# InteractiveComputerGraphics/stark

Measured on AMD Instinct MI355X. Metric: Newton-steps/s, higher is better.
Workload: dtype f64

## Files before the change

stark_amd/csrc/api.cpp:

```cpp
#include <algorithm>
#include <chrono>
#include <cstring>
#include <cstdio>
#include <cstdlib>
#include <string>

#include "dist.hpp"
#include "engine.hpp"
#include "forces.hpp"
#include "../../include/mistark_contact.h"

using namespace mistark;

#define API_BEGIN        \
    if (!ctx) return -1; \
    int _ret = 0;        \
    (void)_ret;          \
    ::mistark::DryScope _dry(ctx->c.dry); \
    try {                \
        if (!ctx->c.dry) (void)hipSetDevice(ctx->c.device);
#define API_END(ret)                   \
    }                                  \
    catch (const std::exception& e)    \
    {                                  \
// ... 445 lines not shown
    API_BEGIN
    ctx->c.touch();
    ctx->c.u_version++;
    Context& c = ctx->c;
    if (potential < 0 || potential >= (int)c.pots.size()) throw Error("bad potential id");
    const int part = dynamic ? 1 : 0;
    if (c.pots[potential].part != part) {
        c.pots[potential].part = part;
        c.layout_dirty = true;
        c.part[0].dirty = c.part[1].dirty = true;
    }
    API_END(0)
}
int mistark_potential_update_connectivity(mistark_ctx* ctx, int potential, const int32_t* conn, int32_t n_elem)
{
    API_BEGIN
    ctx->c.touch_potential(potential);
    Context& c = ctx->c;
    if (potential < 0 || potential >= (int)c.pots.size()) throw Error("bad potential id");
    if (n_elem < 0) throw Error("bad connectivity shape");
    Potential& P = c.pots[potential];
    P.n_elem = n_elem;
    P.conn_host.assign(conn, conn + (size_t)n_elem * P.conn_stride);
    P.conn_dirty = true;
    c.layout_dirty = true;
    API_END(0)
}

int64_t mistark_ndofs(mistark_ctx* ctx)
{
    if (!ctx) return -1;
    int64_t n = 0;
    for (auto& s : ctx->c.dof_sets) n += s.n;
    return n;
}
int mistark_get_dofs(mistark_ctx* ctx, double* u_host)
{
    API_BEGIN
    Context& c = ctx->c;
    prepare(c);
    MS_CHECK(hipMemcpyAsync(u_host, c.u.p, (size_t)c.ndofs * sizeof(double), hipMemcpyDeviceToHost, c.stream));
    MS_CHECK(hipStreamSynchronize(c.stream));
    API_END(0)
}
int mistark_set_dofs(mistark_ctx* ctx, const double* u_host)
{
    API_BEGIN
    ctx->c.touch();
    ctx->c.u_version++;
    Context& c = ctx->c;
    prepare(c);
    MS_CHECK(hipMemcpyAsync(c.u.p, u_host, (size_t)c.ndofs * sizeof(double), hipMemcpyHostToDevice, c.stream));
    MS_CHECK(hipStreamSynchronize(c.stream));
    API_END(0)
}
int64_t mistark_custom_emit(const char* name, const int32_t* strides, int32_t n_bindings, const int32_t* in_dof, const int32_t* ops, const double* constants, int32_t n_ops,
                            int32_t n_inputs, const int32_t* cond_ops, const double* cond_constants, int32_t n_cond_ops, int32_t n_blocks, int32_t compile, char* out, int64_t cap)
{
    try {
        if (!name || !strides || !in_dof || !ops || !constants) throw Error("mistark_custom_emit: null argument");
        size_t code = 0;
        const std::string src = custom_emit_source(name, strides, n_bindings, in_dof, ops, constants, n_ops, n_inputs, cond_ops, cond_constants, n_cond_ops, n_blocks, compile != 0, &code);
        if (out && cap > 0) std::snprintf(out, (size_t)cap, "%s", src.c_str());
        return compile ? (int64_t)code : (int64_t)src.size();
    } catch (const std::exception& e) {
        if (out && cap > 0) std::snprintf(out, (size_t)cap, "%s", e.what());
        return -1;
    }
}
int mistark_get_counter(mistark_ctx* ctx, const char* name, int64_t* out)
{
    API_BEGIN
    Context& c = ctx->c;
    if (!name || !out) throw Error("mistark_get_counter: null argument");
    const std::string n = name;
    if (n == "multi_pgh_launches") *out = c.n_multi_pgh;
    else if (n == "dof_skips_verified") *out = c.n_dof_skips_verified;
    else if (n == "rtc_builds") *out = c.n_rtc_builds;
    else if (n == "custom_kernel_us") *out = (int64_t)c.custom_kernel_us;
    else if (n == "rtc_launches") *out = c.n_rtc_launches;
    else if (n == "rtc_build_ms") *out = (int64_t)(1e3 * c.t_rtc_builds);
    else if (n == "fused_solves") *out = c.n_fused_solves;
    else if (n == "unfused_solves") *out = c.n_unfused_solves;
    else if (n == "evt_tet_us") *out = (int64_t)c.evt_sum[1];
    else if (n == "evt_small_us") *out = (int64_t)c.evt_sum[2];
    else if (n == "evt_gather_us") *out = (int64_t)c.evt_sum[3];
    else if (n == "evt_main_us") *out = (int64_t)c.evt_sum[4];
    else if (n == "evt_pattern_us") *out = (int64_t)c.evt_sum[5];
    else if (n == "evt_n") *out = c.evt_n;
    else if (n == "eval_pgh_issue_us") *out = (int64_t)(1e6 * c.t_eval_issue);
    else if (n == "eval_pgh_wait_us") *out = (int64_t)(1e6 * c.t_eval_wait);
    else if (n == "contact_searches") *out = contact_searches(c, false);
    else if (n == "contact_repeated_searches") *out = contact_searches(c, true);
    else if (n == "ccd_queries") *out = contact_ccd_counter(c, 0);
    else if (n == "ccd_skipped_pairs") *out = contact_ccd_counter(c, 1);
    else if (n == "ccd_capped_pairs") *out = contact_ccd_counter(c, 2);
    else if (n == "ccd_rounds") *out = contact_ccd_counter(c, 3);
    else if (n == "ccd_pad_bound_pairs") *out = contact_ccd_counter(c, 4);
    else if (n == "asm_short_slots_0" || n == "asm_short_slots_1") { ensure_pattern(c); const BsrPart& m = c.part[n.back() - '0']; *out = m.nnzb - m.n_long - m.n_vlong; }
    else if (n == "asm_long_slots_0" || n == "asm_long_slots_1") { ensure_pattern(c); *out = c.part[n.back() - '0'].n_long; }
    else if (n == "asm_vlong_slots_0" || n == "asm_vlong_slots_1") { ensure_pattern(c); *out = c.part[n.back() - '0'].n_vlong; }
    else if (n == "force_readouts") *out = c.n_force_readouts;
    else if (n == "force_long_rows") *out = force_long_rows(c);
    else if (n == "stress_readouts") *out = c.n_stress_readouts;
    else if (n == "stress_long_rows") *out = stress_long_rows(c);
    else if (n == "budget_readouts") *out = c.n_budget_readouts;
    else if (n == "budget_chunks") *out = c.n_budget_chunks;
    else if (n == "constraint_reports") *out = c.n_constraint_reports;
    else if (n == "constraint_report_chunks") *out = c.n_constraint_chunks;
    else if (n == "bending_reports") *out = c.n_bending_reports;
    else if (n == "bending_report_long_rows") *out = bending_long_rows(c);
    else if (n == "bending_report_chunks") *out = c.n_bending_chunks;
    else if (n == "spectrum_reports") *out = c.n_spectrum_reports;
    else if (n == "spectrum_report_long_rows") *out = spectrum_long_rows(c);
    else if (n == "spectrum_report_chunks") *out = c.n_spectrum_chunks;
    else if (n == "linsys_reports") *out = c.n_linsys_reports;
    else if (n == "wrench_reports") *out = c.n_wrench_reports;
    else if (n == "wrench_long_rows") *out = wrench_long_rows(c);
    else if (n == "contact_reports") *out = c.n_contact_reports;
    else if (n == "contact_report_long_rows") *out = contact_report_long_rows(c);
    else if (n == "friction_reports") *out = c.n_friction_reports;
    else if (n == "friction_report_long_rows") *out = friction_report_long_rows(c);
    else if (n == "llt_path") *out = c.llt_last_path;
    else if (n == "llt_panel_rows") *out = c.llt_last_panel_rows;
    else if (n == "llt_panels") *out = c.llt_last_panels;
    else if (n == "llt_fronts") *out = c.llt_last_fronts;
    else throw Error("mistark_get_counter: unknown counter '" + n + "'");
    API_END(0)
}
int mistark_dofs_to_host_arrays(mistark_ctx* ctx)
{
    API_BEGIN
    Context& c = ctx->c;
    prepare(c);
    for (auto& s : c.dof_sets)
        if (s.n > 0) MS_CHECK(hipMemcpyAsync(s.host, c.u.p + s.offset, s.n * sizeof(double), hipMemcpyDeviceToHost, c.stream));
    MS_CHECK(hipStreamSynchronize(c.stream));
    c.u_host_version = c.u_version;
    API_END(0)
}
int mistark_dofs_to_host_arrays_if_changed(mistark_ctx* ctx)
{
    API_BEGIN
    Context& c = ctx->c;
    prepare(c);
    if (c.u_host_version != c.u_version) {
        for (auto& s : c.dof_sets)
            if (s.n > 0) MS_CHECK(hipMemcpyAsync(s.host, c.u.p + s.offset, s.n * sizeof(double), hipMemcpyDeviceToHost, c.stream));
        MS_CHECK(hipStreamSynchronize(c.stream));
        c.u_host_version = c.u_version;
    } else {
        static const bool verify = [] { const char* e = std::getenv("MISTARK_VERIFY_DOF_SKIP"); return e && e[0] == '1'; }();
        if (verify) {
            std::vector<double> tmp;
            for (auto& s : c.dof_sets) {
                if (s.n <= 0) continue;
                tmp.resize((size_t)s.n);
                MS_CHECK(hipMemcpyAsync(tmp.data(), c.u.p + s.offset, s.n * sizeof(double), hipMemcpyDeviceToHost, c.stream));
                MS_CHECK(hipStreamSynchronize(c.stream));
                if (std::memcmp(tmp.data(), s.host, (size_t)s.n * sizeof(double)) != 0)
                    throw Error("mistark_dofs_to_host_arrays_if_changed: the transfer was skipped (version " + std::to_string(c.u_version) + ") but DoF set '" + s.label +
                                "' differs between the device and the caller's array: a writer of the DoF vector did not bump Context::u_version");
            }
            c.n_dof_skips_verified++;
        }
    }
// ... 769 lines not shown
    } catch (const std::exception& e) {
        comm->last_error = e.what();
        return -1;
    }
}
int mistark_rccl_allreduce_bench(int device, int rank, int world, const char unique_id[128], int64_t n_big, int reps, double* out, char* err, int err_len)
{
    if (!unique_id || !out) return -1;
    try {
        rccl_allreduce_bench(device, rank, world, unique_id, (size_t)std::max<int64_t>(n_big, 0), reps, out);
        return 0;
    } catch (const std::exception& e) {
        if (err && err_len > 0) std::snprintf(err, (size_t)err_len, "%s", e.what());
        return -1;
    }
}
int mistark_dist_fused_bench(mistark_ctx* ctx, int n_launches, double* out)
{
    API_BEGIN
    Context& c = ctx->c;
    if (c.world < 2 || !c.coll || !c.coll->ipc()) throw Error("mistark_dist_fused_bench: ranks that exchange through windows only");
    if (!out || n_launches <= 0) throw Error("mistark_dist_fused_bench: bad arguments");
    fused_pcg_replay(c, n_launches, &out[0], &out[1]);
    API_END(0)
}
mistark_local_group* mistark_local_group_create(int world)
{
    if (world < 1) return nullptr;
    auto* g = new mistark_local_group();
    g->g = std::make_shared<LocalGroup>(world);
    return g;
}
void mistark_local_group_destroy(mistark_local_group* g) { delete g; }
int mistark_dist_init_local(mistark_ctx* ctx, mistark_local_group* group, int rank)
{
    API_BEGIN
    if (!group) throw Error("null group");
    set_dist(ctx->c, rank, group->g->world, group->g->world > 1 ? make_local_collective(group->g, rank, ctx->c.device) : nullptr);
    API_END(0)
}

int mistark_set_option(mistark_ctx* ctx, const char* name, int value)
{
    API_BEGIN
    const std::string n = name ? name : "";
    if (n == "force_generic") {
        ctx->c.force_generic = value != 0;
        ctx->c.layout_dirty = true;
    }
    else if (n == "generic_contact") ctx->c.generic_contact = value != 0;
    else if (n == "no_eval_prelaunch") ctx->c.no_eval_prelaunch = value != 0;
    else if (n == "no_multi_eval_p") ctx->c.no_multi_eval_p = value != 0;
    else if (n == "no_multi_eval_pgh") ctx->c.no_multi_eval_pgh = value != 0;
    else if (n == "llt_multifrontal") ctx->c.llt_multifrontal = value;
    else if (n == "llt_no_coords") { ctx->c.llt_no_coords = value != 0; ctx->c.llt_mf_pattern_version = 0; }
    else if (n == "generic_inertia") ctx->c.generic_inertia = value != 0;
    else if (n == "contact_closed_min_lanes") ctx->c.contact_closed_min_lanes = value;
    else if (n == "atomic_assembly") ctx->c.atomic_assembly = value != 0;
    else if (n == "spmv_grid_cap") ctx->c.spmv_grid_cap = value;
    else if (n == "spmv_nt") ctx->c.spmv_nt = value;
    else if (n == "custom_rtc") ctx->c.custom_rtc = value;
    else if (n == "custom_timing") ctx->c.custom_timing = value;
    else if (n == "pcg_batch") ctx->c.pcg_batch = value;
    else if (n == "lazy_hessians") ctx->c.lazy_allowed = value != 0;
    else if (n == "lazy_eval") ctx->c.lazy_eval = value != 0;
    else if (n == "no_pattern_overlap") ctx->c.no_pattern_overlap = value != 0;
    else if (n == "no_eval_overlap") ctx->c.no_eval_overlap = value != 0;
    else if (n == "no_eager_assembly") ctx->c.no_eager_assembly = value != 0;
    else if (n == "no_sym_gather") ctx->c.no_sym_gather = value != 0;
    else if (n == "no_split_gather") ctx->c.no_split_gather = value != 0;
    else if (n == "no_bounded_pattern") { ctx->c.no_bounded_pattern = value != 0; ctx->c.part[1].dirty = true; }
    else if (n == "no_grad_gather") { ctx->c.no_grad_gather = value != 0; ctx->c.layout_dirty = true; }

    else if (n == "spmv_variant") ctx->c.spmv_variant = value;
    else if (n == "proj_variant") ctx->c.proj_variant = value;
    else if (n == "no_contact_cache") ctx->c.no_contact_cache = value != 0;
    else if (n == "no_sharded_search") ctx->c.no_sharded_search = value != 0;
    else if (n == "no_row_order") { ctx->c.no_row_order = value != 0; ctx->c.perm_sig.clear(); ctx->c.layout_dirty = true; }
    else if (n == "row_order") { ctx->c.row_order_mode = value; ctx->c.perm_sig.clear(); ctx->c.layout_dirty = true; }
    else if (n == "atomic_projection") ctx->c.atomic_projection = value != 0;
    else if (n == "no_dyn_pool") { ctx->c.no_dyn_pool = value != 0; ctx->c.layout_dirty = true; }
    else if (n == "no_halo_subset") { ctx->c.no_halo_subset = value != 0; ctx->c.cg_mask_pattern = 0; }
    else if (n == "cg_variant") ctx->c.cg_variant = value;
    else if (n == "no_fused_pcg") ctx->c.no_fused_pcg = value != 0;
    else if (n == "spmv_chunk_tiles") {
        if (value < 0 || value > 64) throw Error("spmv_chunk_tiles: 0 (automatic) .. 64");
        ctx->c.spmv_chunk_tiles = value;
        ctx->c.part[0].dirty = true;
    }
    else throw Error("unknown option '" + n + "'");
    API_END(0)
}

int mistark_sync(mistark_ctx* ctx)
{
    API_BEGIN
    MS_CHECK(hipStreamSynchronize(ctx->c.stream));
    API_END(0)
}
int mistark_spmv_bench(mistark_ctx* ctx, int n_launches, double* avg_us)
{
    API_BEGIN
    const double us = spmv_bench(ctx->c, n_launches);
    if (avg_us) *avg_us = us;
    API_END(0)
}

int mistark_spmv_event_overhead(mistark_ctx* ctx, double* avg_ms)
{
    API_BEGIN
    Context& c = ctx->c;
    if (avg_ms) *avg_ms = c.spmv_n > 0 ? c.spmv_empty_ms_sum / (double)c.spmv_n : 0.0;
    API_END(0)
}
int mistark_spmv_device_clock(mistark_ctx* ctx, double* avg_ms, int64_t* n)
{
    API_BEGIN
    Context& c = ctx->c;
    int khz = 0;
    MS_CHECK(hipDeviceGetAttribute(&khz, hipDeviceAttributeWallClockRate, c.device));
    if (khz <= 0) throw Error("spmv_device_clock: the device reports no wall clock rate");
    if (avg_ms) *avg_ms = c.spmv_clk_n > 0 ? c.spmv_clk_ticks / (double)c.spmv_clk_n / (double)khz : 0.0;
    if (n) *n = c.spmv_clk_n;
    API_END(0)
}
int mistark_spmv_timing(mistark_ctx* ctx, int reset, double* avg_ms, int64_t* n, double* bytes_per_launch)
{
    API_BEGIN
    Context& c = ctx->c;
    if (avg_ms) *avg_ms = c.spmv_n > 0 ? c.spmv_ms_sum / (double)c.spmv_n : 0.0;
    if (n) *n = c.spmv_n;
    if (bytes_per_launch)
        *bytes_per_launch = (double)(c.part[0].nnzb + c.part[1].nnzb) * 40.0 + ((double)c.nbr + 1.0) * 8.0 + 48.0 * (double)c.nbr + 56.0 * (double)c.part[1].n_rows;
    if (reset) {
        c.spmv_ms_sum = 0.0;
        c.spmv_empty_ms_sum = 0.0;
        c.spmv_n = 0;
        c.spmv_clk_ticks = 0.0;
        c.spmv_clk_n = 0;
        c.time_spmv = reset > 0;
    }
    API_END(0)
}

}

namespace mistark {
int force_potentials_by_prefix(mistark_ctx* ctx, const std::string& prefix, std::vector<int32_t>& out)
{
    API_BEGIN
    out.clear();
    for (size_t p = 0; p < ctx->c.pots.size(); p++)
        if (ctx->c.pots[p].name.compare(0, prefix.size(), prefix) == 0) out.push_back((int32_t)p);
    API_END(0)
}
int force_record(mistark_ctx* ctx, int slot, const std::vector<int32_t>& pots, double scale)
{
    API_BEGIN
    force_record_slot(ctx->c, slot, pots.data(), (int32_t)pots.size(), false, scale);
    API_END(0)
}
int force_fetch(mistark_ctx* ctx, int slot, double* f_host, int64_t ndofs)
{
    API_BEGIN
    force_fetch_slot(ctx->c, slot, f_host, ndofs);
    API_END(0)
// ... 160 lines not shown
```

stark_amd/csrc/engine.hpp:

```cpp
#pragma once
#include <algorithm>
#include <cstdlib>
#include <hip/hip_runtime.h>

#include <cstdint>
#include <cstdio>
#include <stdexcept>
#include <map>
#include <string>
#include <vector>

#include <memory>

#include "../../include/mistark.h"

#include "potargs.hpp"

namespace mistark {

struct Error : std::runtime_error
{
    using std::runtime_error::runtime_error;
};

// ... 535 lines not shown
    std::vector<ConstraintReportSet> cnr_slots;
    struct ConstraintPlan
    {
        DevBuf<uint32_t> items;
        DevBuf<int32_t> chunks;
        uint64_t conn_version = 0;
        int n_elem = -1, n_groups = -1;
        int64_t n_chunks = 0;
    };
    std::map<int, ConstraintPlan> cnr_plans;
    DevBuf<double> cnr_tol, cnr_partial;
    int64_t n_constraint_reports = 0;
    int64_t n_constraint_chunks = 0;

    DevBuf<double> bdr_rec, bdr_out, bdr_groups, bdr_thr, bdr_partial;
    DevBuf<uint32_t> bdr_key, bdr_key_alt, bdr_val, bdr_val_alt;
    DevBuf<uint32_t> bdr_stat;
    DevBuf<unsigned char> bdr_desc;
    DevBuf<uint8_t> bdr_cub_tmp;
    struct BendingPlan
    {
        DevBuf<uint32_t> items;
        DevBuf<int32_t> chunks;
        uint64_t conn_version = 0;
        int n_elem = -1, n_groups = -1;
        int64_t n_chunks = 0;
    };
    std::map<int, BendingPlan> bdr_plans;
    struct BendingSlot
    {
        DevBuf<double> rec, nodal, groups[2];
        int64_t N = -1;
        int64_t n_rows[2] = {0, 0}, col0[2] = {0, 0};
        int32_t n_groups = 0;
        int64_t nbr = 0;
    };
    BendingSlot bdr_slot;
    int64_t n_bending_reports = 0;
    int64_t n_bending_chunks = 0;
    bool bdr_stat_valid = false;

    DevBuf<double> wr_pool, wr_elemE, wr_f, wr_rec, wr_out;
    DevBuf<uint32_t> wr_key, wr_key_alt, wr_val, wr_val_alt;
    DevBuf<uint32_t> wr_stat;
    DevBuf<unsigned char> wr_desc;
    DevBuf<uint8_t> wr_cub_tmp, wr_active;
    DevBuf<int32_t> wr_ids, wr_count;
    int wr_stat_families = 0;
    int32_t wr_out_families = 0, wr_out_bodies = 0;
    int64_t n_wrench_reports = 0;

    DevBuf<double> spr_rec, spr_spec, spr_H, spr_gpool, spr_elemE, spr_nodal, spr_partial, spr_pot;
    DevBuf<uint32_t> spr_key, spr_key_alt, spr_val, spr_val_alt;
    DevBuf<uint32_t> spr_stat;
    DevBuf<unsigned char> spr_desc, spr_sdesc;
    DevBuf<uint8_t> spr_cub_tmp;
    DevBuf<int32_t> spr_chunks;
    struct SpectrumSlot
    {
        DevBuf<double> rec, nodal, pot;
        std::vector<int> slot_of;
        std::vector<int64_t> col0, n_elem;
        int64_t N = -1;
        int64_t nbr = 0;
    };
    SpectrumSlot spr_slot;
    int64_t n_spectrum_reports = 0;
    int64_t n_spectrum_chunks = 0;
    bool spr_stat_valid = false;

    DevBuf<double> lsr_V, lsr_w, lsr_t, lsr_y, lsr_part, lsr_c, lsr_ctrl, lsr_L, lsr_diag, lsr_nodal, lsr_q;
    DevBuf<uint8_t> lsr_nz;
    DevBuf<int32_t> lsr_cols;
    int64_t n_linsys_reports = 0;
    struct LinsysSlot
    {
        bool valid = false;
        double rec[16] = {0};
        double low_row = -1.0, low_share = 0.0, high_row = -1.0, high_share = 0.0;
    };
    LinsysSlot lsr_slot;

    int last_cg_iters = 0;
    int64_t n_projected_total = 0;

    ~Context();
};

void direct_mf_destroy(void* multifrontal);
void fetch(Context& c, void* dst_host, const void* src_dev, size_t bytes);
void h2d_staged(Context& c, void* dst_dev, const void* src_host, size_t bytes);
constexpr int FILL_BATCH_MAX = 8;
struct FillQueue
{
    hipStream_t stream;
    void* ptr[FILL_BATCH_MAX];
    size_t words[FILL_BATCH_MAX];
    uint32_t value[FILL_BATCH_MAX];
    int n = 0;
    explicit FillQueue(hipStream_t s) : stream(s) {}
    ~FillQueue() { flush(); }
    void add(void* p, int byte_value, size_t bytes);
    void flush();
};
void fill_async(hipStream_t stream, void* p, int byte_value, size_t bytes);
void copy_async(hipStream_t stream, void* dst, const void* src, size_t bytes);
void prepare(Context& c);
void eval_prelaunch(Context& c, int mode, bool lazy);
void shard_prepare(Context& c);
void shard_halo(Context& c, double* v_local);
void shard_halo_global(Context& c, double* v_global);
void shard_gather_global(Context& c, const double* v_local, double* v_global);
void shard_to_local(Context& c, const double* v_global, double* v_local, bool with_ghosts);
void shard_allgather_scalars(Context& c, const double* mine, int n, double* all_host);
double shard_sum(Context& c, double mine);
void shard_check(Context& c);
struct ElemTable
{
    const int32_t* rows;
    int64_t n_elem;
    int nb;
};
void rcb_partition_rows(int64_t n_block_rows, int world, const double* xyz, const std::vector<int64_t>& weight, std::vector<int32_t>& owner);
void graph_partition_rows(int64_t n_block_rows, int world, const std::vector<ElemTable>& tables, const uint8_t* hub, std::vector<int32_t>& owner);
void static_graph_order(Context& c, std::vector<int32_t>& rows_in_order);
void ensure_pattern(Context& c);
void contact_destroy(struct ContactSystem* cs);
int64_t contact_searches(const Context& c, bool repeated);
int64_t contact_ccd_counter(const Context& c, int which);
int64_t contact_sharded_searches(const Context& c);
void contact_shared_rows(Context& c, std::vector<int32_t>& rows);
struct ContactReportView
{
    const int32_t *cv_src, *cv_mesh, *tri, *tri_mesh, *edge, *edge_mesh, *mesh_kind;
    const double *thick, *k, *X_rest, *rb_xloc;
    const uint64_t* keys;
    int64_t n_keys;
    int bounds[22];
    int n_mesh, n_v, n_t, n_e;
    int prim_bits;
    const std::vector<int32_t>*h_tri, *h_cv_src, *h_cv_mesh;
};
void contact_report_view(Context& c, ContactReportView& v, bool sizes_only);
void contact_report_positions(Context& c, double* X_dev);
void contact_report_sizes(Context& c, int64_t* n_rows, int64_t* n_vertices, int32_t* n_groups);
void contact_report_run(Context& c, int set);
void contact_report_rows(Context& c, int set, int32_t* rows_i, double* rows_d, int64_t* n_rows);
void contact_report_vertices(Context& c, int set, double* out, int32_t* group, int32_t* source_index, int64_t* n_vertices);
void contact_report_pairs(Context& c, int set, double* out, int32_t* n_groups);
int64_t contact_report_long_rows(Context& c);
struct FrictionReportView
{
    struct Table
    {
        const int32_t* conn = nullptr;
        const double *T = nullptr, *mu = nullptr, *fn = nullptr, *bary = nullptr;
        int stride = 0, nbary = 0, start = 0, n = 0;
    };
    const int32_t *cv_src, *cv_mesh, *tri, *tri_mesh, *edge, *edge_mesh, *mesh_kind, *mesh_idx;
    const double *v1, *rb_v1, *rb_w1, *rb_q0, *rb_xloc;
    const uint64_t* keys;
    int64_t n_keys;
    Table tables[14];
    double dt, epsv;
    int n_mesh, n_v, n_t, n_e, prim_bits;
    const std::vector<int32_t>*h_tri, *h_cv_src, *h_cv_mesh;
};
void friction_report_view(Context& c, FrictionReportView& v, bool sizes_only);
void friction_report_sizes(Context& c, int64_t* n_rows, int64_t* n_vertices, int32_t* n_groups);
void friction_report_run(Context& c, int set);
void friction_report_rows(Context& c, int set, int32_t* rows_i, double* rows_d, int64_t* n_rows);
void friction_report_vertices(Context& c, int set, double* out, int32_t* group, int32_t* source_index, int64_t* n_vertices);
void friction_report_pairs(Context& c, int set, double* out, int32_t* n_groups);
int64_t friction_report_long_rows(Context& c);
int register_potential(Context& c, const char* name, const int32_t* conn, int32_t n_elem, int32_t conn_stride, const mistark_binding* bindings, int32_t n_bindings);
void eval(Context& c, int mode, double* E, double* grad_host, double* grad_max_abs = nullptr, bool lazy = false);
void reduce_dot_and_max_abs(Context& c, const double* a, const double* b, int64_t n, double* dot, double* max_abs_a);
void project(Context& c, double eps, int mirroring, const uint8_t* active_host, bool by_gradient, double threshold, int* all_active,
             int64_t* n_projected_now, int64_t* n_changed_now);
void assemble(Context& c);
void build_preconditioner(Context& c);
double spmv_bench(Context& c, int n);
void rows_from_solver(Context& c, const double* v_solver, double* v_caller);
void rows_to_solver(Context& c, const double* v_caller, double* v_solver);
void fused_pcg_replay(Context& c, int n_launches, double* s_us, double* v_us);
void spmv_device(Context& c, const double* x, double* y, const double* pdot, double* partials);
void pcg(Context& c, const double* rhs_dev, double abs_tol, double rel_tol, int max_iter, int stop_on_indef, mistark_pcg_info* info, double rhs_scale = 1.0);
bool direct_llt(Context& c, const double* rhs_dev, double* x_dev);
std::shared_ptr<CustomProgram> make_custom_program(const std::string& name, const int32_t* strides, int n_bindings, const int32_t* ops, const double* consts, int n_ops, int n_inputs,
                                                   const int32_t* cond_ops, const double* cond_consts, int n_cond_ops);
void custom_program_set_summation(CustomProgram& G, const std::string& name, int first_input, int stride, int n_iterations, const double* data);
void launch_eval_custom(Context& c, Potential& P, int mode);
void h2d_small(Context& c, void* dst_dev, const void* src_host, size_t bytes);
double reduce_max_abs(Context& c, const double* v, int64_t n);
double reduce_dot(Context& c, const double* a, const double* b, int64_t n);
void vec_axpby(Context& c, double* dst, double a, const double* x, double b, const double* y, int64_t n);
void vec_fill(Context& c, double* dst, double v, int64_t n);
void vec_neg(Context& c, double* dst, const double* x, int64_t n);
void launch_force_elements(Context& c, const Potential& P, double* pool, double* scratchE);
bool force_readout(Context& c, const int32_t* pots, int32_t n, bool all, double scale, double* f_dev);
void force_elements_host(Context& c, int pot, double scale, double* out, int32_t* block_rows, int64_t* n_elem, int32_t* nb);
void force_nodal_host(Context& c, const int32_t* pots, int32_t n, double scale, double* f_host);
void force_resultant_host(Context& c, const int32_t* pots, int32_t n, double scale, const int32_t* rows, int64_t n_rows, const double* pos_host, const double* about, double* out);
int64_t force_long_rows(Context& c);
void force_record_slot(Context& c, int slot, const int32_t* pots, int32_t n, bool all, double scale);
void force_fetch_slot(Context& c, int slot, double* f_host, int64_t n);
void stress_elements_host(Context& c, int pot, double* out, int64_t* n_elem, int32_t* kind);
void stress_nodal_host(Context& c, const int32_t* pots, int32_t n, double* out_host);
int64_t stress_long_rows(Context& c);
void stress_record_kind(Context& c, int kind);
void stress_fetch_elements(Context& c, int kind, double* out, int64_t* n_elem);
void stress_fetch_nodal(Context& c, int kind, double* out, int64_t n_rows);
std::vector<int> select_potentials(Context& c, const int32_t* pots, int32_t n, bool all, const char* who);
void launch_energy_elements(Context& c, const Potential& P, double* scratchE);
void budget_energies(Context& c, const int32_t* pots, int32_t n, double* out_host, int slot);
void budget_inertia(Context& c, int pot, const double* about, int32_t n_groups, double* out_host, int slot);
void budget_rigid(Context& c, int t0, int q0, int v1, int w1, int mass, int J_loc, int32_t n_bodies, const double* about, double* out_host, int slot);
void budget_fetch_slot(Context& c, int slot, double* out_host, int64_t n);
void constraint_rows_host(Context& c, int pot, const double* tolerance, int32_t n_groups, double* out, double* aux, int32_t* ids, int64_t* n_rows, int32_t* kind);
void constraint_groups_host(Context& c, int pot, const double* tolerance, int32_t n_groups, const double* about, double* out);
void constraint_record_kind(Context& c, int pot, const double* tolerance, int32_t n_groups, const double* about, int32_t* kind);
void constraint_fetch_kind(Context& c, int kind, double* out, double* aux, int32_t* ids, double* groups, int64_t* n_rows, int32_t* n_groups);
void bending_rows_host(Context& c, int pot, const double* threshold, int32_t n_groups, double* out, int64_t* n_rows, int32_t* kind);
void bending_nodal_host(Context& c, const int32_t* pots, int32_t n, double* out_host);
void bending_groups_host(Context& c, int pot, const double* threshold, int32_t n_groups, double* out);
int64_t bending_long_rows(Context& c);
void bending_record_step(Context& c, int pot_complete, int pot_flat, const double* threshold, int32_t n_groups);
void bending_fetch_kind(Context& c, int kind, double* rows, double* groups, int64_t* n_rows, int32_t* n_groups);
void bending_fetch_nodal(Context& c, double* out, int64_t n_rows);
void launch_hessian_elements(Context& c, const Potential& P, double* Hpool, double* scratchE, double* scratch_gpool);
void spectrum_rows_host(Context& c, int pot, int source, double eps, double* out, double* spectrum, int64_t* n_elem, int32_t* nb);
void spectrum_nodal_host(Context& c, const int32_t* pots, int32_t n, int source, double eps, double* out_host);
void spectrum_pots_host(Context& c, const int32_t* pots, int32_t n, int source, double eps, double* out);
int64_t spectrum_long_rows(Context& c);
void spectrum_record_step(Context& c, const int32_t* pots, int32_t n, double eps);
void spectrum_fetch_summary(Context& c, int32_t n, double* pots_out, double* nodal_out, int64_t n_rows);
void spectrum_fetch_rows(Context& c, int32_t index, double* rows, int64_t* n_rows);
void linsys_report_host(Context& c, int op, int m, const double* start_host, double* out, double* ritz, double* tri, int32_t* k_out);
void linsys_modes_host(Context& c, int op, int m, const double* start_host, const int32_t* which, int32_t n_which, double* x_host, double* nodal, double* mode);
void linsys_potential_shares_host(Context& c, int op, int m, const double* start_host, int32_t which, const int32_t* pots, int32_t n, double* out);
void linsys_record_step(Context& c, int op, int m);
void linsys_fetch(Context& c, double* rec16, double* rows4);
void wrench_rows_host(Context& c, int pot, int v1, int w1, int t0, int q0, int32_t n_bodies, double* out, int32_t* ids, int64_t* n_rows);
void wrench_bodies_host(Context& c, const int32_t* families, const int32_t* family_start, int32_t n_families, int v1, int w1, int t0, int q0, int32_t n_bodies, const double* about,
                        double* out, int32_t* count);
int64_t wrench_long_rows(Context& c);
void wrench_record_step(Context& c, const std::vector<std::vector<int32_t>>& families, const std::vector<char>& all, int v1, int w1, int t0, int q0, int32_t n_bodies,
                        const double* about);
void wrench_fetch_step(Context& c, int32_t n_families, int32_t n_bodies, double* out, int32_t* count);
struct InertiaBindings
{
    const double *dt = nullptr, *gravity = nullptr;
};
InertiaBindings inertia_bindings(const Context& c);
int find_kind(const char* name);
int kind_nb(int kind);
int kind_nbind(int kind);
void kind_strides(int kind, int* out);
const char* kind_name(int kind);
int n_kinds();

int newton_solve(Context& c, const mistark_newton_settings& s, const mistark_newton_callbacks* cb, mistark_newton_stats& st);
// ... 10 lines not shown
```

stark_amd/csrc/newton.cpp:

```cpp
#include <algorithm>
#include <chrono>
#include <cmath>
#include <cstdio>
#include <cstdlib>
#include <limits>

#include "engine.hpp"

namespace mistark {

namespace {
struct Timer
{
    double& acc;
    std::chrono::steady_clock::time_point t0;
    explicit Timer(double& a) : acc(a), t0(std::chrono::steady_clock::now()) {}
    ~Timer() { acc += std::chrono::duration<double>(std::chrono::steady_clock::now() - t0).count(); }
};
enum Stage { ST_EVAL_PGH, ST_EVAL_P, ST_ASSEMBLY, ST_PROJECT, ST_SOLVE, ST_OTHER, ST_COUNT };
struct GpuStages
{
    Context& c;
    std::vector<std::pair<int, size_t>> marks;
    size_t used = 0;
    explicit GpuStages(Context& ctx) : c(ctx) {}
    void mark(int stage)
    {
        if (used == c.stage_ev.size()) {
            hipEvent_t e;
            MS_CHECK(hipEventCreate(&e));
            c.stage_ev.push_back(e);
        }
        MS_CHECK(hipEventRecord(c.stage_ev[used], c.stream));
        marks.emplace_back(stage, used++);
    }
    void collect(double* seconds )
    {
        if (marks.empty()) return;
        MS_CHECK(hipEventSynchronize(c.stage_ev[marks.back().second]));
        for (size_t i = 0; i + 1 < marks.size(); i++) {
            float ms = 0.f;
            if (hipEventElapsedTime(&ms, c.stage_ev[marks[i].second], c.stage_ev[marks[i + 1].second]) == hipSuccess) seconds[marks[i].first] += 1e-3 * ms;
        }
    }
};
}

int newton_solve(Context& c, const mistark_newton_settings& s, const mistark_newton_callbacks* cb, mistark_newton_stats& st)
{
    Timer t_total(st.t_total);
    prepare(c);
    GpuStages gs(c);
    double stage_s[ST_COUNT] = {0, 0, 0, 0, 0, 0};
    const int64_t ndofs = c.ndofs;
    auto sync = [&]() { MS_CHECK(hipStreamSynchronize(c.stream)); };
    auto call_void = [&](void (*f)(void*)) {
        if (cb && f) {
            Timer t(st.t_callbacks);
            sync();
            f(cb->user);
        }
    };
    auto call_bool = [&](int (*f)(void*), bool def) -> bool {
        if (cb && f) {
            Timer t(st.t_callbacks);
            sync();
            return f(cb->user) != 0;
        }
        return def;
    };

    double E0 = 0.0, du_dot_grad = 0.0, res_0 = std::numeric_limits<double>::max();
    static const bool trace = std::getenv("MISTARK_NEWTON_TRACE") != nullptr;
    int result = MISTARK_RUNNING;
    int pdn_countdown = 0;
    double ppn_threshold = -1.0;

    c.newton_log.clear();
    if (!call_bool(cb ? cb->is_initial_state_valid : nullptr, true)) result = MISTARK_INVALID_INITIAL_STATE;

    int it = -1;
    while (result == MISTARK_RUNNING) {
        it++;
        if (it == s.max_iterations) {
            result = s.max_iterations_as_success ? MISTARK_SUCCESSFUL : MISTARK_TOO_MANY_ITERATIONS;
            break;
        }
        const bool lazy = c.lazy_allowed && (s.projection_mode == MISTARK_PROJ_PROGRESSIVE || s.projection_mode == MISTARK_PROJ_NEWTON) && s.linear_solver != MISTARK_SOLVER_DIRECT_LLT;
        if (cb && cb->before_energy_evaluation) eval_prelaunch(c, MISTARK_EVAL_P_G_H, lazy);
        call_void(cb ? cb->before_energy_evaluation : nullptr);
        double residual = 0.0;
        {
            gs.mark(ST_EVAL_PGH);
            eval(c, MISTARK_EVAL_P_G_H, &E0, nullptr, &residual, lazy);
            st.n_evaluations++;
            gs.mark(ST_OTHER);
        }
        if (it == 0) res_0 = residual;
        c.newton_log.push_back(mistark_newton_iteration{});
        c.newton_log.back().residual = residual;
        if (trace) std::fprintf(stderr, "         %d. r0: %.2e | \n", it, residual);
        if (!std::isfinite(residual) || !std::isfinite(E0)) {
            result = MISTARK_LINEAR_SYSTEM_SOLVE_FAILURE;
            break;
        }
        if (residual < s.bailout_residual) {
            result = MISTARK_SUCCESSFUL;
            break;
        }
        if (it >= s.min_iterations) {
            if (residual < s.residual_tolerance_abs) {
                result = MISTARK_SUCCESSFUL;
                break;
            }
            if (it > 0 && residual / res_0 < s.residual_tolerance_rel) {
                result = MISTARK_SUCCESSFUL;
                break;
            }
        }

        double du_max_solved = 0.0;
        bool assembled = false;
        bool solved = false;
        while (!solved) {
            bool all_projected = false;
            if (s.projection_mode == MISTARK_PROJ_PROGRESSIVE && !assembled) {
                gs.mark(ST_ASSEMBLY);
                assemble(c);
                assembled = true;
            }
            bool reassemble = !assembled;
            {
                gs.mark(ST_PROJECT);
                switch (s.projection_mode) {
                    case MISTARK_PROJ_NEWTON: break;
                    case MISTARK_PROJ_PROJECTED_NEWTON: {
                        int64_t np = 0;
                        project(c, s.projection_eps, s.project_to_pd_use_mirroring, nullptr, false, 0.0, nullptr, &np, nullptr);
                        all_projected = true;
                        break;
                    }
                    case MISTARK_PROJ_ON_DEMAND:
                        if (pdn_countdown > 0) {
                            int64_t np = 0;
                            project(c, s.projection_eps, s.project_to_pd_use_mirroring, nullptr, false, 0.0, nullptr, &np, nullptr);
                            all_projected = true;
                        }
                        break;
                    case MISTARK_PROJ_PROGRESSIVE:
                        if (ppn_threshold > 0.0) {
                            if (ppn_threshold < 1e-12) ppn_threshold = 0.0;
                            int all_active = 0;
                            int64_t np = 0;
                            project(c, s.projection_eps, s.project_to_pd_use_mirroring, nullptr, true, ppn_threshold, &all_active, &np, nullptr);
                            all_projected = all_active != 0;
                        }
                        break;
                    default: throw Error("unknown projection mode");
                }
            }
            if (reassemble || !c.matrix_current) {
                gs.mark(ST_ASSEMBLY);
                assemble(c);
                assembled = true;
            }

            mistark_pcg_info info{};
            {
                gs.mark(ST_SOLVE);
                const double forcing = std::min(1e-2, residual * std::min(0.5, std::sqrt(residual)));
                const double abs_tol = std::max(forcing, s.cg_abs_tolerance);
                if (s.linear_solver == MISTARK_SOLVER_DIRECT_LLT) {
                    vec_neg(c, c.tmp_a.p, c.grad.p, ndofs);
                    info.converged = direct_llt(c, c.tmp_a.p, c.du.p) ? 1 : 0;
                } else if (c.world > 1) {
                    vec_neg(c, c.tmp_a.p, c.grad.p, ndofs);
                    pcg(c, c.tmp_a.p, abs_tol, s.cg_rel_tolerance, s.cg_max_iterations, s.cg_stop_on_indefiniteness, &info);
                } else {
                    pcg(c, c.grad.p, abs_tol, s.cg_rel_tolerance, s.cg_max_iterations, s.cg_stop_on_indefiniteness, &info, -1.0);
                }
                st.cg_iterations += info.n_iterations;
                st.n_linear_solves++;
                c.newton_log.back().linear_solves++;
                c.newton_log.back().cg_iterations_last = info.n_iterations;
                c.newton_log.back().cg_iterations_all += info.n_iterations;
                if (trace) std::fprintf(stderr, "            solve: #CG %5d | tol %.2e | %s%s| ppn threshold %.2e\n", info.n_iterations, abs_tol, info.converged ? "converged " : "",
                                        info.found_indefiniteness ? "indefinite " : "", ppn_threshold);
                gs.mark(ST_OTHER);
            }
            const bool ok = info.converged != 0;
            const bool can_project_more = (s.projection_mode != MISTARK_PROJ_NEWTON) && !all_projected;
            if (!ok && !can_project_more) {
                result = MISTARK_LINEAR_SYSTEM_SOLVE_FAILURE;
                break;
            }
            bool descends = false;
            if (ok) {
                reduce_dot_and_max_abs(c, c.du.p, c.grad.p, ndofs, &du_dot_grad, &du_max_solved);
                descends = du_dot_grad < 0.0;
                if (!descends && !can_project_more) {
                    result = MISTARK_STEP_DOES_NOT_DESCEND;
                    break;
                }
            }
            if (ok && descends) {
                solved = true;
                break;
            }
            if (s.projection_mode == MISTARK_PROJ_ON_DEMAND) pdn_countdown = s.project_on_demand_countdown;
            else if (s.projection_mode == MISTARK_PROJ_PROGRESSIVE) {
                if (ppn_threshold < 0.0) ppn_threshold = residual;
                ppn_threshold *= s.ppn_tightening_factor;
            }
        }
        if (result != MISTARK_RUNNING) break;

        if (s.projection_mode == MISTARK_PROJ_ON_DEMAND) pdn_countdown--;
        else if (s.projection_mode == MISTARK_PROJ_PROGRESSIVE) ppn_threshold *= s.ppn_release_factor;

        st.n_hessians += (int64_t)c.n_elem_total;
        st.n_projected_hessians += c.n_projected_total;
        {
            mistark_newton_iteration& rec = c.newton_log.back();
            rec.logged = 1;
            rec.n_hessians = (int64_t)c.n_elem_total;
            rec.n_projected_hessians = c.n_projected_total;
            rec.du_max = du_max_solved;
        }

        double du_max = du_max_solved;
        if (trace) std::fprintf(stderr, "            du: %.1e | E0: %.10e\n", du_max, E0);
        if (it >= s.min_iterations && du_max < s.step_tolerance) {
            result = MISTARK_SUCCESSFUL;
            break;
        }

        const int ls0[4] = {st.ls_cap_iterations, st.ls_max_iterations, st.ls_inv_iterations, st.ls_bt_iterations};
        {
            double* u0 = c.tmp_b.p;
            copy_async(c.stream, u0, c.u.p, (size_t)ndofs * sizeof(double));
            auto apply = [&](double step) { vec_axpby(c, c.u.p, 1.0, u0, step, c.du.p, ndofs); };
            double retraction = 1.0;
            if (du_max > s.step_cap) {
                retraction *= s.step_cap / du_max;
                vec_axpby(c, c.du.p, retraction, c.du.p, 0.0, nullptr, ndofs);
                du_max = s.step_cap;
                st.ls_cap_iterations++;
            }
            double max_step = 1.0;
            if (cb && cb->max_allowed_step) {
                Timer t(st.t_callbacks);
                sync();
                max_step = std::min(1.0, cb->max_allowed_step(cb->user));
            }
            if (max_step < 1.0) {
                retraction *= max_step;
                vec_axpby(c, c.du.p, max_step, c.du.p, 0.0, nullptr, ndofs);
                du_max *= max_step;
                st.ls_max_iterations++;
            }
            double step = 1.0;
            apply(step);
            int inv_it = 0;
            for (; inv_it < s.max_backtracking_invalid_state_iterations; ++inv_it) {
                if (call_bool(cb ? cb->is_intermediate_state_valid : nullptr, true)) break;
                step *= 0.5;
                apply(step);
                st.ls_inv_iterations++;
            }
            if (inv_it == s.max_backtracking_invalid_state_iterations) {
                call_void(cb ? cb->on_intermediate_state_invalid : nullptr);
                result = MISTARK_TOO_MANY_INVALID_INTERMEDIATE_ITERATIONS;
            } else if (s.enable_armijo_backtracking) {
                const double expected = s.line_search_armijo_beta * du_dot_grad * retraction;
                double E_threshold = E0 + expected * step;
                double E1 = 0.0;
                int k = 0;
                for (; k < s.max_backtracking_armijo_iterations; ++k) {
                    if (cb && cb->before_energy_evaluation) eval_prelaunch(c, MISTARK_EVAL_P, false);
                    call_void(cb ? cb->before_energy_evaluation : nullptr);
                    {
// ... 48 lines not shown
```

stark_amd/csrc/project.hip:

```cpp
#include "kernels_common.hpp"

namespace mistark {


struct SelDesc
{
    const int32_t* conn;
    const uint32_t* elem_list;
    const int32_t* lrow;
    uint8_t* is_projected;
    uint32_t* list;
    uint32_t* list_e;
    int conn_stride, e_count, NB, counter, first_block, n_own;
    int dof_col[MAX_NB], dof_row_off[MAX_NB];
};
__global__ __launch_bounds__(BLOCK) void k_project_select_multi(const SelDesc* __restrict__ D, int n_desc, const uint8_t* __restrict__ active_blocks, int64_t* __restrict__ counters)
{
    __shared__ int s_k;
    if (threadIdx.x == 0) {
        int k = 0;
        while (k + 1 < n_desc && (int)blockIdx.x >= D[k + 1].first_block) k++;
        s_k = k;
    }
    __syncthreads();
// ... 761 lines not shown
                else hipLaunchKernelGGL((k_project_eig_ti<3>), grid_ti, b_ti, 0, stream, H, n_key, n_pool, compact, list, nl, eps, mirroring, sos, vals, c.counters.p);
                continue;
            }
            const dim3 grid(((nl + epw - 1) / epw + 3) / 4);
            switch (P.NB) {
                case 1: hipLaunchKernelGGL((k_project_eig_cols<1>), grid, b, 0, stream, H, n_key, n_pool, compact, list, nl, eps, mirroring, sos, vals, c.counters.p); break;
                case 2: hipLaunchKernelGGL((k_project_eig_cols<2>), grid, b, 0, stream, H, n_key, n_pool, compact, list, nl, eps, mirroring, sos, vals, c.counters.p); break;
                case 3: hipLaunchKernelGGL((k_project_eig_cols<3>), grid, b, 0, stream, H, n_key, n_pool, compact, list, nl, eps, mirroring, sos, vals, c.counters.p); break;
                case 4: hipLaunchKernelGGL((k_project_eig_cols<4>), grid, b, 0, stream, H, n_key, n_pool, compact, list, nl, eps, mirroring, sos, vals, c.counters.p); break;
                case 5: hipLaunchKernelGGL((k_project_eig_cols<5>), grid, b, 0, stream, H, n_key, n_pool, compact, list, nl, eps, mirroring, sos, vals, c.counters.p); break;
                default: hipLaunchKernelGGL((k_project_eig_cols<6>), grid, b, 0, stream, H, n_key, n_pool, compact, list, nl, eps, mirroring, sos, vals, c.counters.p); break;
            }
            continue;
        }
        switch (P.NB) {
            case 1: hipLaunchKernelGGL((k_project_eig<1>), g, b, 0, stream, H, n_key, n_pool, compact, list, nl, eps, mirroring, sos, vals, c.counters.p); break;
            case 2: hipLaunchKernelGGL((k_project_eig<2>), g, b, 0, stream, H, n_key, n_pool, compact, list, nl, eps, mirroring, sos, vals, c.counters.p); break;
            case 3: hipLaunchKernelGGL((k_project_eig<3>), g, b, 0, stream, H, n_key, n_pool, compact, list, nl, eps, mirroring, sos, vals, c.counters.p); break;
            case 4: hipLaunchKernelGGL((k_project_eig<4>), g, b, 0, stream, H, n_key, n_pool, compact, list, nl, eps, mirroring, sos, vals, c.counters.p); break;
            case 5: hipLaunchKernelGGL((k_project_eig<5>), g, b, 0, stream, H, n_key, n_pool, compact, list, nl, eps, mirroring, sos, vals, c.counters.p); break;
            case 6: hipLaunchKernelGGL((k_project_eig<6>), g, b, 0, stream, H, n_key, n_pool, compact, list, nl, eps, mirroring, sos, vals, c.counters.p); break;
            case 7: hipLaunchKernelGGL((k_project_eig<7>), g, b, 0, stream, H, n_key, n_pool, compact, list, nl, eps, mirroring, sos, vals, c.counters.p); break;
            case 8: hipLaunchKernelGGL((k_project_eig<8>), g, b, 0, stream, H, n_key, n_pool, compact, list, nl, eps, mirroring, sos, vals, c.counters.p); break;
            default: throw Error("project: unsupported block count");
        }
    }
    flush();
    if (marks.empty()) return;
    for (int part = 0; part < 2; part++)
        if (mark_part[part]) {
            BsrPart& m = c.part[part];
            const size_t n_pos = (size_t)std::max<int64_t>(m.ntiles * 64, m.nnzb) + 4;
            if (m.slot_dirty.cap < n_pos) {
                m.slot_dirty.ensure(n_pos);
                MS_CHECK(hipMemsetAsync(m.slot_dirty.p, 0, m.slot_dirty.cap, c.stream));
            }
        }
    MarkBatch mb;
    mb.n = 0;
    int blocks = 0;
    auto flush_marks = [&]() {
        if (mb.n > 0) hipLaunchKernelGGL(k_proj_mark, dim3(blocks), dim3(BLOCK), 0, c.stream, mb);
        mb.n = 0;
        blocks = 0;
    };
    for (const Mark& k : marks) {
        Potential& P = c.pots[(size_t)k.pot];
        BsrPart& m = c.part[P.part];
        const bool lazy = k.Hc != nullptr;
        if (k.nl <= 0) continue;
        if (mb.n == MARK_BATCH) flush_marks();
        mb.d[mb.n++] = MarkDesc{k.list, (const uint32_t*)(m.slot_of_src.p + P.kp_off), m.slot_dirty.p, k.Hc, lazy ? c.elemHf.p + P.hf_off : (float*)nullptr, k.nl, P.NB, P.n_key,
                                k.n_pool_c, P.n_pool_f, blocks};
        blocks += grid_for((int64_t)k.nl * P.NB * P.NB);
    }
    flush_marks();
    for (int part = 0; part < 2; part++)
        if (mark_part[part]) {
            BsrPart& m = c.part[part];
            gather_part(c, part, m.slot_dirty.p);
            fill_async(c.stream, m.slot_dirty.p, 0, ((size_t)std::max<int64_t>(m.ntiles * 64, m.nnzb) + 3) & ~(size_t)3);
        }
}
void project(Context& c, double eps, int mirroring, const uint8_t* active_host, bool by_gradient, double threshold, int* all_active, int64_t* n_projected_now,
             int64_t* n_changed_now)
{
    if (c.static_assembled) MS_CHECK(hipStreamWaitEvent(c.stream, c.aux_ev[2], 0));
    ensure_pattern(c);
    if (!c.have_hessians) throw Error("project: no element Hessians (call eval with MISTARK_EVAL_P_G_H first)");
    project_select(c, active_host, by_gradient, threshold);
    int64_t h[128];
    fetch(c, h, c.counters.p, sizeof(h));
    int64_t n_inactive = h[2], n_selected = h[3];
    if (c.world > 1) {
        double mine[2] = {(double)h[2], (double)h[3]}, all[2 * 64];
        shard_allgather_scalars(c, mine, 2, all);
        n_inactive = n_selected = 0;
        for (int r = 0; r < c.world; r++) {
            n_inactive += (int64_t)all[2 * r];
            n_selected += (int64_t)all[2 * r + 1];
        }
    }
    project_selected(c, h, eps, mirroring);
    c.n_projected_total += n_selected;
    if (n_projected_now) *n_projected_now = n_selected;
    if (n_changed_now) {
        int64_t h2[2];
        fetch(c, h2, c.counters.p, sizeof(h2));
        *n_changed_now = h2[1];
    }
    if (all_active) *all_active = by_gradient ? (n_inactive == 0) : (active_host == nullptr);
}


}
```

Baseline: 215.3.

## Replay unchanged PCG solves and skip empty projection selection in progressive projection

```diff
diff --git a/stark_amd/csrc/api.cpp b/stark_amd/csrc/api.cpp
--- a/stark_amd/csrc/api.cpp
+++ b/stark_amd/csrc/api.cpp
@@ -551,6 +551,11 @@
     else if (n == "rtc_build_ms") *out = (int64_t)(1e3 * c.t_rtc_builds);
     else if (n == "fused_solves") *out = c.n_fused_solves;
     else if (n == "unfused_solves") *out = c.n_unfused_solves;
+    else if (n == "solves_replayed") *out = c.n_solves_replayed;
+    else if (n == "cg_iterations_replayed") *out = c.n_cg_iterations_replayed;
+    else if (n == "solve_replays_verified") *out = c.n_solve_replays_verified;
+    else if (n == "selections_skipped") *out = c.n_selections_skipped;
+    else if (n == "pcg_solves") *out = c.pcg_epoch;
     else if (n == "evt_tet_us") *out = (int64_t)c.evt_sum[1];
     else if (n == "evt_small_us") *out = (int64_t)c.evt_sum[2];
     else if (n == "evt_gather_us") *out = (int64_t)c.evt_sum[3];
@@ -1486,6 +1491,8 @@
     else if (n == "no_dyn_pool") { ctx->c.no_dyn_pool = value != 0; ctx->c.layout_dirty = true; }
     else if (n == "no_halo_subset") { ctx->c.no_halo_subset = value != 0; ctx->c.cg_mask_pattern = 0; }
     else if (n == "cg_variant") ctx->c.cg_variant = value;
+    else if (n == "no_solve_replay") ctx->c.no_solve_replay = value != 0;
+    else if (n == "verify_solve_replay") ctx->c.verify_solve_replay = value != 0;
     else if (n == "no_fused_pcg") ctx->c.no_fused_pcg = value != 0;
     else if (n == "spmv_chunk_tiles") {
         if (value < 0 || value > 64) throw Error("spmv_chunk_tiles: 0 (automatic) .. 64");
diff --git a/stark_amd/csrc/engine.hpp b/stark_amd/csrc/engine.hpp
--- a/stark_amd/csrc/engine.hpp
+++ b/stark_amd/csrc/engine.hpp
@@ -641,6 +641,12 @@
     LinsysSlot lsr_slot;
 
     int last_cg_iters = 0;
+    bool no_solve_replay = false, verify_solve_replay = false;
+    int64_t n_solves_replayed = 0;
+    int64_t n_cg_iterations_replayed = 0;
+    int64_t n_solve_replays_verified = 0;
+    int64_t n_selections_skipped = 0;
+    int64_t n_inactive_last = 0;
     int64_t n_projected_total = 0;
 
     ~Context();
@@ -737,6 +743,7 @@
 void reduce_dot_and_max_abs(Context& c, const double* a, const double* b, int64_t n, double* dot, double* max_abs_a);
 void project(Context& c, double eps, int mirroring, const uint8_t* active_host, bool by_gradient, double threshold, int* all_active,
              int64_t* n_projected_now, int64_t* n_changed_now);
+void project_none_active(Context& c, int* all_active, int64_t* n_projected_now);
 void assemble(Context& c);
 void build_preconditioner(Context& c);
 double spmv_bench(Context& c, int n);
diff --git a/stark_amd/csrc/newton.cpp b/stark_amd/csrc/newton.cpp
--- a/stark_amd/csrc/newton.cpp
+++ b/stark_amd/csrc/newton.cpp
@@ -3,7 +3,10 @@
 #include <cmath>
 #include <cstdio>
 #include <cstdlib>
+#include <cstring>
 #include <limits>
+#include <string>
+#include <vector>
 
 #include "engine.hpp"
 
@@ -122,12 +125,23 @@
         double du_max_solved = 0.0;
         bool assembled = false;
         bool solved = false;
+        struct
+        {
+            bool valid = false, has_dot = false;
+            mistark_pcg_info info{};
+            double abs_tol = 0.0, du_dot_grad = 0.0, du_max = 0.0;
+        } last_solve;
+        int round_no = -1;
         while (!solved) {
+            round_no++;
+            int64_t n_projected_now = -1;
+            bool matrix_touched = false;
             bool all_projected = false;
             if (s.projection_mode == MISTARK_PROJ_PROGRESSIVE && !assembled) {
                 gs.mark(ST_ASSEMBLY);
                 assemble(c);
                 assembled = true;
+                matrix_touched = true;
             }
             bool reassemble = !assembled;
             {
@@ -152,8 +166,18 @@
                             if (ppn_threshold < 1e-12) ppn_threshold = 0.0;
                             int all_active = 0;
                             int64_t np = 0;
-                            project(c, s.projection_eps, s.project_to_pd_use_mirroring, nullptr, true, ppn_threshold, &all_active, &np, nullptr);
+                            const bool none_active = c.world == 1 && ppn_threshold > residual && !c.no_solve_replay;
+                            if (none_active && !c.verify_solve_replay) {
+                                project_none_active(c, &all_active, &np);
+                                c.n_selections_skipped++;
+                            } else {
+                                project(c, s.projection_eps, s.project_to_pd_use_mirroring, nullptr, true, ppn_threshold, &all_active, &np, nullptr);
+                                if (none_active && (np != 0 || c.n_inactive_last != c.nbr || (all_active != 0) != (c.nbr == 0)))
+                                    throw Error("verify_solve_replay: Newton iteration " + std::to_string(it) + ", round " + std::to_string(round_no) + ": a threshold above the residual selected " +
+                                                std::to_string(np) + " elements and left " + std::to_string(c.n_inactive_last) + " of " + std::to_string(c.nbr) + " rows inactive");
+                            }
                             all_projected = all_active != 0;
+                            n_projected_now = np;
                         }
                         break;
                     default: throw Error("unknown projection mode");
@@ -163,14 +187,38 @@
                 gs.mark(ST_ASSEMBLY);
                 assemble(c);
                 assembled = true;
+                matrix_touched = true;
             }
 
             mistark_pcg_info info{};
+            bool replayed = false;
             {
                 gs.mark(ST_SOLVE);
                 const double forcing = std::min(1e-2, residual * std::min(0.5, std::sqrt(residual)));
                 const double abs_tol = std::max(forcing, s.cg_abs_tolerance);
-                if (s.linear_solver == MISTARK_SOLVER_DIRECT_LLT) {
+                const bool same_system = last_solve.valid && s.projection_mode == MISTARK_PROJ_PROGRESSIVE && s.linear_solver != MISTARK_SOLVER_DIRECT_LLT && c.world == 1 &&
+                                         n_projected_now == 0 && !matrix_touched && c.matrix_current && abs_tol == last_solve.abs_tol && !c.no_solve_replay;
+                if (!same_system) last_solve.valid = false;
+                if (same_system && !c.verify_solve_replay) {
+                    info = last_solve.info;
+                    replayed = true;
+                    c.n_solves_replayed++;
+                    c.n_cg_iterations_replayed += info.n_iterations;
+                } else if (same_system) {
+                    std::vector<double> du_before((size_t)ndofs), du_after((size_t)ndofs);
+                    fetch(c, du_before.data(), c.du.p, (size_t)ndofs * sizeof(double));
+                    pcg(c, c.grad.p, abs_tol, s.cg_rel_tolerance, s.cg_max_iterations, s.cg_stop_on_indefiniteness, &info, -1.0);
+                    fetch(c, du_after.data(), c.du.p, (size_t)ndofs * sizeof(double));
+                    const mistark_pcg_info& r = last_solve.info;
+                    const bool same_info = info.n_iterations == r.n_iterations && info.converged == r.converged && info.found_indefiniteness == r.found_indefiniteness &&
+                                           std::memcmp(&info.error, &r.error, sizeof(info.error)) == 0;
+                    if (!same_info || std::memcmp(du_before.data(), du_after.data(), (size_t)ndofs * sizeof(double)) != 0)
+                        throw Error("verify_solve_replay: Newton iteration " + std::to_string(it) + ", round " + std::to_string(round_no) + ": the solve the replay stands for ended " +
+                                    (same_info ? "with another du" : "in " + std::to_string(info.n_iterations) + " iterations (converged " + std::to_string(info.converged) + ", indefinite " +
+                                                                         std::to_string(info.found_indefiniteness) + "), the recorded one in " + std::to_string(r.n_iterations) + " (" +
+                                                                         std::to_string(r.converged) + ", " + std::to_string(r.found_indefiniteness) + ")"));
+                    c.n_solve_replays_verified++;
+                } else if (s.linear_solver == MISTARK_SOLVER_DIRECT_LLT) {
                     vec_neg(c, c.tmp_a.p, c.grad.p, ndofs);
                     info.converged = direct_llt(c, c.tmp_a.p, c.du.p) ? 1 : 0;
                 } else if (c.world > 1) {
@@ -184,8 +232,14 @@
                 c.newton_log.back().linear_solves++;
                 c.newton_log.back().cg_iterations_last = info.n_iterations;
                 c.newton_log.back().cg_iterations_all += info.n_iterations;
-                if (trace) std::fprintf(stderr, "            solve: #CG %5d | tol %.2e | %s%s| ppn threshold %.2e\n", info.n_iterations, abs_tol, info.converged ? "converged " : "",
-                                        info.found_indefiniteness ? "indefinite " : "", ppn_threshold);
+                if (trace) std::fprintf(stderr, "            solve: #CG %5d | tol %.2e | %s%s%s| ppn threshold %.2e\n", info.n_iterations, abs_tol, info.converged ? "converged " : "",
+                                        info.found_indefiniteness ? "indefinite " : "", replayed ? "replayed " : "", ppn_threshold);
+                if (!replayed && !same_system) {
+                    last_solve.valid = true;
+                    last_solve.has_dot = false;
+                    last_solve.info = info;
+                    last_solve.abs_tol = abs_tol;
+                }
                 gs.mark(ST_OTHER);
             }
             const bool ok = info.converged != 0;
@@ -196,7 +250,17 @@
             }
             bool descends = false;
             if (ok) {
-                reduce_dot_and_max_abs(c, c.du.p, c.grad.p, ndofs, &du_dot_grad, &du_max_solved);
+                if (replayed && last_solve.has_dot) {
+                    du_dot_grad = last_solve.du_dot_grad;
+                    du_max_solved = last_solve.du_max;
+                } else {
+                    reduce_dot_and_max_abs(c, c.du.p, c.grad.p, ndofs, &du_dot_grad, &du_max_solved);
+                    if (last_solve.valid && last_solve.has_dot && (std::memcmp(&du_dot_grad, &last_solve.du_dot_grad, sizeof(double)) != 0 || std::memcmp(&du_max_solved, &last_solve.du_max, sizeof(double)) != 0))
+                        throw Error("verify_solve_replay: Newton iteration " + std::to_string(it) + ", round " + std::to_string(round_no) + ": du.grad or max |du| differ from the recorded ones");
+                    last_solve.has_dot = true;
+                    last_solve.du_dot_grad = du_dot_grad;
+                    last_solve.du_max = du_max_solved;
+                }
                 descends = du_dot_grad < 0.0;
                 if (!descends && !can_project_more) {
                     result = MISTARK_STEP_DOES_NOT_DESCEND;
diff --git a/stark_amd/csrc/project.hip b/stark_amd/csrc/project.hip
--- a/stark_amd/csrc/project.hip
+++ b/stark_amd/csrc/project.hip
@@ -867,6 +867,7 @@
         }
     }
     project_selected(c, h, eps, mirroring);
+    c.n_inactive_last = n_inactive;
     c.n_projected_total += n_selected;
     if (n_projected_now) *n_projected_now = n_selected;
     if (n_changed_now) {
@@ -876,6 +877,15 @@
     }
     if (all_active) *all_active = by_gradient ? (n_inactive == 0) : (active_host == nullptr);
 }
-
-
-}
+void project_none_active(Context& c, int* all_active, int64_t* n_projected_now)
+{
+    if (c.static_assembled) MS_CHECK(hipStreamWaitEvent(c.stream, c.aux_ev[2], 0));
+    ensure_pattern(c);
+    if (!c.have_hessians) throw Error("project: no element Hessians (call eval with MISTARK_EVAL_P_G_H first)");
+    c.n_inactive_last = c.nbr;
+    if (n_projected_now) *n_projected_now = 0;
+    if (all_active) *all_active = c.nbr == 0;
+}
+
+
+}
```

After: 217.9, median of 3. No clear change (+1.2%).
